# yqtianust/FeatureNet

Hardware: AMD Instinct MI355X
Metric: samples/sec (64^3 voxel, 24-class) train (higher is better)
Workload: dtype bf16; 1 GPU; model=FeatureNet-3D, global_batch=128, per_gpu_batch=128, input=64^3x1 voxels, classes=24, parallelism=dp1, impl=native, optimizer=adam, graph=True

## Files before the change

featurenet_amd/csrc/kernels/bind.cpp:

```cpp
#include <hip/hip_runtime.h>
#include <pybind11/pybind11.h>
#include <pybind11/stl.h>

#include <stdexcept>
#include <string>
#include <vector>

namespace py = pybind11;

extern "C" {
int fn_igemm_fwd(const void*, const void*, const float*, void*, float*, const int*, const int*, long long, int, int,
                 int, int, int, hipStream_t, float*, int);
int fn_igemm_fwd_splits(long long, int, int);
int fn_igemm_fwd_mblocks(long long);
int fn_conv_halo(const void*, const void*, const float*, void*, float*, const int*, const int*, int, int, int*,
                 hipStream_t);
long long fn_conv_halo_lds(const int*, int);
int fn_conv_halo_workers(const int*, int);
int fn_pw_fwd(const void*, const void*, const float*, void*, long long, int, int, int, hipStream_t, const float*,
              const float*, int, const void*, const float*, const float*, float*, int);
int fn_seghead_part_len();
int fn_part_reduce(const float*, float*, long long, int, int, hipStream_t);
int fn_seghead_blocks(long long);
int fn_seghead_loss(const void*, const float*, const float*, const void*, const float*, const void*, void*, float*,
// ... 66 lines not shown
int fn_dense_wgrad_slices(int, int, int);
int fn_s2d_weight_map(const float*, float*, const int*, int, hipStream_t);
int fn_subpixel_wmap(const float*, float*, int, int, int, hipStream_t);
int fn_halo_pack_w(const float*, void*, int, int, int, int, int, int, int, hipStream_t);
int fn_igemm_pack_w(const float*, void*, int, int, int, int, int, int, int, int, int, hipStream_t);
int fn_pack_w_multi(const long long*, int, hipStream_t);
int fn_igemm_wgrad(const void*, const void*, float*, const int*, const int*, long long, int, int, int, int,
                   hipStream_t, int, int, const void*, int, float*, int, float*);
long long fn_igemm_wgrad_part(int, int, int, int, int, int, int);
int fn_colstats(const void*, const void*, const float*, const float*, const float*, const float*, float*, long long,
                int, int, int, int, hipStream_t);
int fn_bn_finalize(const float*, int, int, double, const float*, const float*, float*, float*, float, float, float*,
                   float*, float*, float*, int, hipStream_t);
int fn_bn_apply(const void*, const float*, const float*, void*, long long, int, int, hipStream_t, void*);
int fn_bn_wdot(const float*, const float*, float*, int, int, int, hipStream_t);
int fn_bn_bwd_prep(const float*, int, const float*, int, int, double, const float*, const float*, const float*,
                   const float*, const float*, const float*, float*, float*, const void*, const void*, long long,
                   hipStream_t);
int fn_bn_bwd_apply_k_blocks(long long, int);
int fn_bn_bwd_apply_k(const void*, const void*, const float*, const float*, const float*, const float*, void*,
                      long long, int, float*, int, hipStream_t);
int fn_bn_bwd_apply(const void*, const void*, const float*, const float*, const float*, const float*, const float*,
                    const float*, void*, long long, int, float, int, hipStream_t);
int fn_bn_bwd_apply_s2d(const void*, const void*, const float*, const float*, const float*, const float*,
                        const float*, const float*, void*, int, int, int, int, int, float, int, hipStream_t);
int fn_pool_fwd(const void*, void*, const float*, const float*, const int*, int, int, int, hipStream_t);
int fn_pool_bwd(const void*, const void*, void*, const float*, const float*, const int*, int, int, int, hipStream_t);
int fn_pool_bwd_stats_blocks(const int*);
int fn_colstats_blocks(long long, int, int, int);
int fn_pool_bn_bwd_apply(const void*, const void*, const float*, const float*, const float*, const float*,
                         const float*, const float*, void*, const int*, int, float, hipStream_t);
int fn_pool_bwd_stats(const void*, const void*, void*, const float*, const float*, const int*, int, float*,
                      hipStream_t);
int fn_softmax_xent_blocks(long long, int);
int fn_upsample2x(const void*, void*, int, int, int, int, int, int, hipStream_t);
int fn_softmax_xent_rows(const void*, int, const long long*, float*, void*, int*, long long, int, float, float,
                         hipStream_t);
int fn_adam_flat_dev(float*, const float*, float*, float*, void*, long long, const float*, int*, int, hipStream_t);
int fn_adam_flat(float*, const float*, float*, float*, void*, long long, float, float, float, float, float, float,
                 float, float, int, hipStream_t);
int fn_sgd_flat(float*, const float*, float*, void*, long long, float, float, float, int, float, hipStream_t);
int fn_bias_act(const void*, const float*, void*, long long, int, int, hipStream_t);
int fn_act_bwd(const void*, const void*, void*, long long, int, hipStream_t);
int fn_dropout(const void*, void*, long long, float, unsigned, unsigned, hipStream_t);
int fn_cast_f32_bf16(const float*, void*, long long, hipStream_t);
int fn_scale_unless_one(void*, int, const float*, long long, hipStream_t);
int fn_copy2(void*, const void*, long long, void*, const void*, long long, hipStream_t);
int fn_cu_occupy(int, int, int, void*, hipStream_t);
int fn_softmax_rows(const float*, float*, long long, int, int, const float*, hipStream_t);
int fn_unpack_bits(const void*, void*, long long, hipStream_t);
int fn_conv_tile(const void*, const void*, const void*, const void*, const void*, const float*, void*, float*,
                 const int*, int, int, int, int, int*, hipStream_t, const void*, const float*, float, void*);
int fn_conv_tile_workers(const int*, int, int);
int fn_conv_tile_slab_rows(const int*, int, int);
void fn_conv_tile_grid_cap(int);
void fn_conv_tile_set_schedule(int);
int fn_conv_tile_schedule();
int fn_conv_tile_f8(const void*, const void*, const void*, const void*, const void*, const float*, const float*, void*,
                    float, const int*, int, int, int, int, int*, hipStream_t, const void*, void*);
int fn_conv_tile_f8_supported(int, int, int);
int fn_conv_wtile(const void*, const void*, float*, float*, const void*, const void*, const void*, const int*, int, int,
                  int*, hipStream_t, const float*, float*, const float*, int);
int fn_conv_wtile_supported(int, int);
int fn_conv_wtile_prologue_built();
int fn_tile_pack_w(const float*, void*, int, int, int, int, int, int, int, int, int, hipStream_t);
int fn_tile_pack_w2(const float*, void*, void*, int, int, int, const int*, const int*, hipStream_t);
// ... 832 lines not shown
  m.def("pool_fwd", [check_pool](uintptr_t x, uintptr_t out, uintptr_t scale, uintptr_t shift, std::vector<int> geom,
                       int is_max, int count_pad, int act, uintptr_t st, std::vector<long long> ext) {
    need(geom, 17, "pool_fwd");
    check_pool(geom, ext, "pool_fwd");
    chk(fn_pool_fwd(P<const void*>(x), P<void*>(out), P<const float*>(scale), P<const float*>(shift), geom.data(),
                    is_max, count_pad, act, S(st)),
        "pool_fwd");
  }, py::arg("x"), py::arg("out"), py::arg("scale"), py::arg("shift"), py::arg("geom"), py::arg("is_max"),
     py::arg("count_pad"), py::arg("act"), py::arg("st"), py::arg("ext") = std::vector<long long>());
  m.def("pool_bwd", [check_pool](uintptr_t dout, uintptr_t x, uintptr_t dx, uintptr_t scale, uintptr_t shift,
                       std::vector<int> geom, int is_max, int count_pad, int act, uintptr_t st,
                       std::vector<long long> ext) {
    need(geom, 17, "pool_bwd");
    check_pool(geom, ext, "pool_bwd");
    chk(fn_pool_bwd(P<const void*>(dout), P<const void*>(x), P<void*>(dx), P<const float*>(scale),
                    P<const float*>(shift), geom.data(), is_max, count_pad, act, S(st)),
        "pool_bwd");
  }, py::arg("dout"), py::arg("x"), py::arg("dx"), py::arg("scale"), py::arg("shift"), py::arg("geom"),
     py::arg("is_max"), py::arg("count_pad"), py::arg("act"), py::arg("st"), py::arg("ext") = std::vector<long long>());
  m.def("pool_bwd_stats_blocks", [](std::vector<int> geom) {
    need(geom, 17, "pool_bwd_stats_blocks");
    return fn_pool_bwd_stats_blocks(geom.data());
  });
  m.def("pool_bwd_stats", [check_pool](uintptr_t dout, uintptr_t x, uintptr_t dx, uintptr_t scale, uintptr_t shift,
                             std::vector<int> geom, int act, uintptr_t part, uintptr_t st, std::vector<long long> ext) {
    need(geom, 17, "pool_bwd_stats");
    check_pool(geom, ext, "pool_bwd_stats");
    fits(ext, 2, 2LL * fn_pool_bwd_stats_blocks(geom.data()) * geom[4], "pool_bwd_stats", "part");
    chk(fn_pool_bwd_stats(P<const void*>(dout), P<const void*>(x), P<void*>(dx), P<const float*>(scale),
                          P<const float*>(shift), geom.data(), act, P<float*>(part), S(st)),
        "pool_bwd_stats");
  }, py::arg("dout"), py::arg("x"), py::arg("dx"), py::arg("scale"), py::arg("shift"), py::arg("geom"),
     py::arg("act"), py::arg("part"), py::arg("st"), py::arg("ext") = std::vector<long long>());
  m.def("pool_bn_bwd_apply", [check_pool](uintptr_t dout, uintptr_t y, uintptr_t scale, uintptr_t shift,
                                uintptr_t mean, uintptr_t invstd, uintptr_t dbeta, uintptr_t dgamma, uintptr_t dy,
                                std::vector<int> geom, int act, float inv_count, uintptr_t st,
                                std::vector<long long> ext) {
    need(geom, 17, "pool_bn_bwd_apply");
    check_pool(geom, ext, "pool_bn_bwd_apply");
    chk(fn_pool_bn_bwd_apply(P<const void*>(dout), P<const void*>(y), P<const float*>(scale), P<const float*>(shift),
                             P<const float*>(mean), P<const float*>(invstd), P<const float*>(dbeta),
                             P<const float*>(dgamma), P<void*>(dy), geom.data(), act, inv_count, S(st)),
        "pool_bn_bwd_apply");
  }, py::arg("dout"), py::arg("y"), py::arg("scale"), py::arg("shift"), py::arg("mean"), py::arg("invstd"),
     py::arg("dbeta"), py::arg("dgamma"), py::arg("dy"), py::arg("geom"), py::arg("act"), py::arg("inv_count"),
     py::arg("st"), py::arg("ext") = std::vector<long long>());
  m.def("upsample2x", [](uintptr_t x, uintptr_t y, int N, int D, int H, int W, int C, int backward, uintptr_t st) {
    chk(fn_upsample2x(P<const void*>(x), P<void*>(y), N, D, H, W, C, backward, S(st)), "upsample2x");
  });
  m.def("softmax_xent_blocks", [](long long B, int NC) { return fn_softmax_xent_blocks(B, NC); });
  m.def("softmax_xent_rows", [](uintptr_t logits, int in_bf16, uintptr_t labels, uintptr_t block_loss,
                                uintptr_t dlogits, uintptr_t correct, long long B, int NC, float gscale,
                                float smoothing, uintptr_t st) {
    chk(fn_softmax_xent_rows(P<const void*>(logits), in_bf16, P<const long long*>(labels), P<float*>(block_loss),
                             P<void*>(dlogits), P<int*>(correct), B, NC, gscale, smoothing, S(st)),
        "softmax_xent_rows");
  });
  m.def("softmax_rows", [](uintptr_t x, uintptr_t y, long long M, int N, int backward, uintptr_t g, uintptr_t st,
                           std::vector<long long> ext) {
    fits(ext, 0, M * N, "softmax_rows", "x");
    fits(ext, 1, M * N, "softmax_rows", "y");
    if (backward) fits(ext, 2, M * N, "softmax_rows", "g");
    chk(fn_softmax_rows(P<const float*>(x), P<float*>(y), M, N, backward, P<const float*>(g), S(st)), "softmax_rows");
  });
  m.def("cu_occupy", [](int nwg, int usec, int lds, uintptr_t sink, uintptr_t st) {
    chk(fn_cu_occupy(nwg, usec, lds, P<void*>(sink), S(st)), "cu_occupy");
// ... 44 lines not shown
```

featurenet_amd/csrc/kernels/bn_pool.hip:

```cpp
#include "common.h"

#include <algorithm>
#include <type_traits>

template <int VW>
__device__ __forceinline__ void block_moments_to_part(const float (&s0)[VW], const float (&s1)[VW], bool active, int C,
                                                      float* __restrict__ part) {
  __shared__ float red[256][2 * VW + 1];
  const int tid = threadIdx.x;
  const int cpr = C / VW, rpp = 256 / cpr;
#pragma unroll
  for (int j = 0; j < VW; ++j) { red[tid][j] = active ? s0[j] : 0.f; red[tid][VW + j] = active ? s1[j] : 0.f; }
  __syncthreads();
  for (int c = tid; c < C; c += 256) {
    const int chk = c / VW, j = c % VW;
    float a = 0.f, b = 0.f;
    for (int i = 0; i < rpp; ++i) { a += red[i * cpr + chk][j]; b += red[i * cpr + chk][VW + j]; }
    part[(long long)blockIdx.x * 2 * C + c] = a;
    part[(long long)blockIdx.x * 2 * C + C + c] = b;
  }
}

template <int VW>
__device__ __forceinline__ void bn_bwd_consts(int c0, const float* __restrict__ scale, const float* __restrict__ shift,
// ... 509 lines not shown
          const int iw = ow * g.sw - g.pw + kw;
          if ((unsigned)iw >= (unsigned)g.W) continue;
          ++cnt;
          const long long base = (((n * g.D + id) * g.H + ih) * (long long)g.W + iw) * g.C + ch * VW;
          if constexpr (VW == 8) {
            Pack8 p;
            p.u = *(const uint4*)(x + base);
#pragma unroll
            for (int j = 0; j < 8; ++j) {
              float v = bf2f(p.e[j]);
              if (scale) v = act_fwd(v * scale[ch * 8 + j] + shift[ch * 8 + j], act);
              accv[j] = is_max ? fmaxf(accv[j], v) : accv[j] + v;
            }
          } else {
            const float v = load_pre(x, base, ch, scale, shift, act);
            accv[0] = is_max ? fmaxf(accv[0], v) : accv[0] + v;
          }
        }
      }
    }
    const float div = count_pad ? (float)(g.KD * g.KH * g.KW) : (float)(cnt > 0 ? cnt : 1);
    const long long ob = i * VW;
    if constexpr (VW == 8) {
      Pack8 p;
#pragma unroll
      for (int j = 0; j < 8; ++j) p.e[j] = f2bf(is_max ? accv[j] : accv[j] / div);
      *(uint4*)(out + ob) = p.u;
    } else {
      out[ob] = f2bf(is_max ? accv[0] : accv[0] / div);
    }
  }
}

template <int KD, int ACT = -1>
__global__ __launch_bounds__(256) void pool2_fwd_kernel(const bf16* __restrict__ x, bf16* __restrict__ out,
                                                        const float* __restrict__ scale, const float* __restrict__ shift,
                                                        PoolGeom g, int is_max, int act, int total) {
  const int actc = ACT >= 0 ? ACT : act;
  const int cpr = g.C >> 3;
  const int ch = threadIdx.x % cpr;
  float sc[8], sh[8];
#pragma unroll
  for (int j = 0; j < 8; ++j) {
    sc[j] = scale ? scale[ch * 8 + j] : 1.f;
    sh[j] = scale ? shift[ch * 8 + j] : 0.f;
  }
  const long long rowW = (long long)g.W * g.C, plane = (long long)g.H * rowW;
  auto origin = [&](int ii) -> long long {
    int t = ii / cpr;
    const int ow = t % g.OW; t /= g.OW;
    const int oh = t % g.OH; t /= g.OH;
    const int od = t % g.OD;
    const int n = t / g.OD;
    return ((long long)(n * g.D + od * KD) * g.H + oh * 2) * rowW + (long long)ow * 2 * g.C + ch * 8;
  };
  auto fetch = [&](long long b0, Pack8* p) {
#pragma unroll
    for (int kd = 0; kd < KD; ++kd)
#pragma unroll
      for (int kh = 0; kh < 2; ++kh)
#pragma unroll
        for (int kw = 0; kw < 2; ++kw) p[(kd * 2 + kh) * 2 + kw].u = *(const uint4*)(x + b0 + kd * plane + kh * rowW + kw * g.C);
  };
  const int stride = gridDim.x * 256;
  int i = blockIdx.x * 256 + threadIdx.x;
  Pack8 p[KD * 4];
  if (i < total) fetch(origin(i), p);
  while (i < total) {
    const int inx = i + stride;
    Pack8 p2[KD * 4];
    fetch(origin(inx < total ? inx : i), p2);
    Pack8 o;
#pragma unroll
    for (int j = 0; j < 8; ++j) {
      float acc = is_max ? -INFINITY : 0.f;
#pragma unroll
      for (int w = 0; w < KD * 4; ++w) {
        float v = bf2f(p[w].e[j]);
        if (scale) v = act_fwd(v * sc[j] + sh[j], actc);
        acc = is_max ? fmaxf(acc, v) : acc + v;
      }
      o.e[j] = f2bf(is_max ? acc : acc * (1.f / (KD * 4)));
    }
    *(uint4*)(out + (long long)i * 8) = o.u;
#pragma unroll
    for (int w = 0; w < KD * 4; ++w) p[w] = p2[w];
    i = inx;
  }
}

template <int VW>
__global__ __launch_bounds__(256) void pool_bwd_kernel(const bf16* __restrict__ dout, const bf16* __restrict__ x,
                                                       bf16* __restrict__ dx, const float* __restrict__ scale,
                                                       const float* __restrict__ shift, PoolGeom g, int is_max,
                                                       int count_pad, int act) {
  const int cpr = g.C / VW;
  const long long total = (long long)g.N * g.D * g.H * g.W * cpr;
  for (long long i = blockIdx.x * 256LL + threadIdx.x; i < total; i += (long long)gridDim.x * 256) {
    const int ch = (int)(i % cpr);
    long long t = i / cpr;
    const int iw = (int)(t % g.W); t /= g.W;
    const int ih = (int)(t % g.H); t /= g.H;
    const int id = (int)(t % g.D);
    const long long n = t / g.D;
    float gacc[VW];
    float self[VW];
#pragma unroll
    for (int j = 0; j < VW; ++j) {
      gacc[j] = 0.f;
      const int c = ch * VW + j;
      self[j] = is_max ? load_pre(x, i * VW + j, c, scale, shift, act) : 0.f;
    }
    const int od0 = max(0, (id + g.pd - g.KD + g.sd) / g.sd), od1 = min(g.OD - 1, (id + g.pd) / g.sd);
    const int oh0 = max(0, (ih + g.ph - g.KH + g.sh) / g.sh), oh1 = min(g.OH - 1, (ih + g.ph) / g.sh);
    const int ow0 = max(0, (iw + g.pw - g.KW + g.sw) / g.sw), ow1 = min(g.OW - 1, (iw + g.pw) / g.sw);
    for (int od = od0; od <= od1; ++od)
      for (int oh = oh0; oh <= oh1; ++oh)
// ... 183 lines not shown
      if (w < win) qy[w].u = *(const uint4*)(y + b0 + wofs[w]);
  };
  const I stride = (I)gridDim.x * 256;
  I i = (I)blockIdx.x * 256 + threadIdx.x;
  Pack8 pg, py[8];
  if (i < total) fetch(i, pg, py);
  while (i < total) {
    const I inx = i + stride;
    Pack8 pg2, py2[8];
    fetch(inx < total ? inx : i, pg2, py2);
#pragma unroll
    for (int j = 0; j < 8; ++j) {
      float best = -INFINITY, yarg = 0.f;
#pragma unroll
      for (int w = 0; w < 8; ++w) {
        if (w < win) {
          const float yv = bf2f(py[w].e[j]);
          const float v = act_fwd(yv * sc[j] + sh[j], actc);
          if (v > best) { best = v; yarg = yv; }
        }
      }
      const float gv = bf2f(pg.e[j]) * act_bwd_from_out(best, actc);
      s0[j] += gv;
      s1[j] += gv * yarg;
    }
    pg = pg2;
#pragma unroll
    for (int w = 0; w < 8; ++w) py[w] = py2[w];
    i = inx;
  }
  block_moments_to_part<8>(s0, s1, true, g.C, part);
}

template <typename I, int ACT = -1>
__global__ __launch_bounds__(256) void pool_bn_bwd_apply_kernel(
    const bf16* __restrict__ dout, const bf16* __restrict__ y, const float* __restrict__ scale,
    const float* __restrict__ shift, const float* __restrict__ mean, const float* __restrict__ invstd,
    const float* __restrict__ dbeta, const float* __restrict__ dgamma, bf16* __restrict__ dy, PoolGeom g, int act,
    float inv_count) {
  const int actc = ACT >= 0 ? ACT : act;
  const int cpr = g.C / 8;
  const I total = (I)g.N * g.OD * g.OH * g.OW * cpr;
  const int win = g.KD * g.KH * g.KW;
  const int ch = (int)(threadIdx.x % cpr);
  float sc[8], sh[8], k2[8], k3[8];
  bn_bwd_consts<8>(ch * 8, scale, shift, mean, invstd, dbeta, dgamma, inv_count, sc, sh, k2, k3);
  I wofs[8];
  pool_win_offsets<I>(g, win, wofs);
  auto origin = [&](I ii) -> I { return pool_win_origin<I>(g, ii, cpr, ch); };
  auto fetch = [&](I ii, I b0, Pack8& q, Pack8* qy) {
    q.u = *(const uint4*)(dout + ii * 8);
#pragma unroll
    for (int w = 0; w < 8; ++w)
      if (w < win) qy[w].u = *(const uint4*)(y + b0 + wofs[w]);
  };
  const I stride = (I)gridDim.x * 256;
  I i = (I)blockIdx.x * 256 + threadIdx.x;
  Pack8 pg, py[8];
  I b0 = 0;
  if (i < total) {
    b0 = origin(i);
    fetch(i, b0, pg, py);
  }
  while (i < total) {
    const I inx = i + stride;
    const I in2 = inx < total ? inx : i;
// ... 186 lines not shown
    const int u = rowlen > 4 * 256 && rowlen <= 5 * 256 ? 5 : (rowlen > 5 * 256 && rowlen <= 8 * 256 ? 8 : 4);
    bool launched = false;
    with_int_of<ACT_RELU, ACT_NONE>(act, [&](auto A) {
      with_int_of<0, 1, 2, 3, 4, 5>(lc, [&](auto L) {
        launched = with_int_of<4, 5, 8>(u, [&](auto U) {
          hipLaunchKernelGGL((bn_bwd_apply_s2d_rows_kernel<A(), L(), U()>), dim3(grid), dim3(256), 0, st,
                             (const bf16*)dz, (const bf16*)y, scale, shift, mean, invstd, dbeta, dgamma, (bf16*)dsh, N,
                             FD, FH, FW, C, inv_count);
        });
      });
    });
    if (!launched) return -2;
    FN_CHECK_LAUNCH();
    return 0;
  }
  with_act(act, [&](auto A) {
    hipLaunchKernelGGL((bn_bwd_apply_s2d_kernel<A()>), dim3(ew_blocks(nvec)), dim3(256), 0, st, (const bf16*)dz,
                       (const bf16*)y, scale, shift, mean, invstd, dbeta, dgamma, (bf16*)dsh, N, FD, FH, FW, C, inv_count);
  });
  FN_CHECK_LAUNCH();
  return 0;
}

static PoolGeom pool_geom(const int* g) {
  PoolGeom p;
  p.N = g[0]; p.D = g[1]; p.H = g[2]; p.W = g[3]; p.C = g[4];
  p.OD = g[5]; p.OH = g[6]; p.OW = g[7];
  p.KD = g[8]; p.KH = g[9]; p.KW = g[10];
  p.sd = g[11]; p.sh = g[12]; p.sw = g[13];
  p.pd = g[14]; p.ph = g[15]; p.pw = g[16];
  return p;
}

extern "C" int fn_pool_fwd(const void* x, void* out, const float* scale, const float* shift, const int* geom17,
                           int is_max, int count_pad, int act, hipStream_t st) {
  PoolGeom g = pool_geom(geom17);
  const long long outs = (long long)g.N * g.OD * g.OH * g.OW;
  const bool win2 = g.KH == 2 && g.KW == 2 && (g.KD == 2 || g.KD == 1) && g.sd == g.KD && g.sh == 2 && g.sw == 2 &&
                    g.pd == 0 && g.ph == 0 && g.pw == 0 && g.D >= g.OD * g.KD && g.H >= g.OH * 2 &&
                    g.W >= g.OW * 2 && chunk_fixed(g.C) && outs * (g.C / 8) + 256LL * 8192 < (1LL << 31);
  if (win2) {
    const int total = (int)(outs * (g.C / 8));
    with_int_of<2, 1>(g.KD, [&](auto K) {
      with_act_rn(scale ? act : ACT_NONE, [&](auto A) {
        static const int res = bn_resident_blocks((const void*)pool2_fwd_kernel<K(), A()>);
        hipLaunchKernelGGL((pool2_fwd_kernel<K(), A()>), dim3(resident_grid((total + 255) / 256, res)), dim3(256), 0,
                           st, (const bf16*)x, (bf16*)out, scale, shift, g, is_max, act, total);
      });
    });
  } else
    with_vw(g.C % 8 == 0, [&](auto VW) {
      hipLaunchKernelGGL(pool_fwd_kernel<VW()>, dim3(ew_blocks(outs * (g.C / VW()))), dim3(256), 0, st, (const bf16*)x,
                         (bf16*)out, scale, shift, g, is_max, count_pad, act);
    });
  FN_CHECK_LAUNCH();
  return 0;
}

static bool pool_i32(const PoolGeom& g) {
  const long long ins = (long long)g.N * g.D * g.H * g.W * g.C;
  const long long outs = (long long)g.N * g.OD * g.OH * g.OW * g.C;
  return ins + 256LL * 8192 * 8 < (1LL << 31) && outs + 256LL * 8192 * 8 < (1LL << 31);
}

static bool pool_tiled(const PoolGeom& g) {
  return g.sd == g.KD && g.sh == g.KH && g.sw == g.KW && g.pd == 0 && g.ph == 0 && g.pw == 0 &&
         g.D == g.OD * g.KD && g.H == g.OH * g.KH && g.W == g.OW * g.KW;
}

static bool pool_bwd_stats_ok(const PoolGeom& g) { return pool_tiled(g) && chunk_fixed(g.C); }

extern "C" int fn_pool_bwd_stats_blocks(const int* geom17) {
  const PoolGeom g = pool_geom(geom17);
  if (!pool_bwd_stats_ok(g)) return 0;
  int res = 0;
  if (g.KD * g.KH * g.KW <= 8) {
    static const int r = bn_resident_blocks((const void*)pool_bn_moments8_kernel<int>);
    res = r;
  }
  return resident_rows(((long long)g.N * g.OD * g.OH * g.OW * (g.C / 8) + 255) / 256, res);
}

extern "C" int fn_pool_bwd_stats(const void* dout, const void* x, void* dx, const float* scale, const float* shift,
                                 const int* geom17, int act, float* part, hipStream_t st) {
  const PoolGeom g = pool_geom(geom17);
  const int nb = fn_pool_bwd_stats_blocks(geom17);
  if (nb <= 0 || !scale || !shift || !part) return -2;
  if (!dx && g.KD * g.KH * g.KW <= 8) {
    with_index(pool_i32(g), [&](auto I) {
      with_act_rn(act, [&](auto A) {
        hipLaunchKernelGGL((pool_bn_moments8_kernel<decltype(I), A()>), dim3(nb), dim3(256), 0, st, (const bf16*)dout,
                           (const bf16*)x, scale, shift, g, act, part);
      });
    });
  } else
    hipLaunchKernelGGL((pool_bwd_tiled_kernel<8, true>), dim3(nb), dim3(256), 0, st, (const bf16*)dout, (const bf16*)x,
                       (bf16*)dx, scale, shift, g, 1, act, part);
  FN_CHECK_LAUNCH();
  return 0;
}

extern "C" int fn_pool_bn_bwd_apply(const void* dout, const void* y, const float* scale, const float* shift,
                                    const float* mean, const float* invstd, const float* dbeta, const float* dgamma,
                                    void* dy, const int* geom17, int act, float inv_count, hipStream_t st) {
  const PoolGeom g = pool_geom(geom17);
  if (!pool_tiled(g) || !chunk_fixed(g.C) || g.KD * g.KH * g.KW > 8) return -2;
  const long long outs = (long long)g.N * g.OD * g.OH * g.OW;
  static const int res = bn_resident_blocks((const void*)pool_bn_bwd_apply_kernel<int>);
  const unsigned nb = resident_grid((outs * (g.C / 8) + 255) / 256, res);
  with_index(pool_i32(g), [&](auto I) {
    with_act_rn(act, [&](auto A) {
      hipLaunchKernelGGL((pool_bn_bwd_apply_kernel<decltype(I), A()>), dim3(nb), dim3(256), 0, st, (const bf16*)dout,
                         (const bf16*)y, scale, shift, mean, invstd, dbeta, dgamma, (bf16*)dy, g, act, inv_count);
    });
  });
  FN_CHECK_LAUNCH();
  return 0;
}

extern "C" int fn_pool_bwd(const void* dout, const void* x, void* dx, const float* scale, const float* shift,
                           const int* geom17, int is_max, int count_pad, int act, hipStream_t st) {
  PoolGeom g = pool_geom(geom17);
  if (pool_tiled(g)) {
    const long long outs = (long long)g.N * g.OD * g.OH * g.OW;
    with_vw(g.C % 8 == 0, [&](auto VW) {
      hipLaunchKernelGGL(pool_bwd_tiled_kernel<VW()>, dim3(ew_blocks(outs * (g.C / VW()))), dim3(256), 0, st,
                         (const bf16*)dout, (const bf16*)x, (bf16*)dx, scale, shift, g, is_max, act);
    });
    FN_CHECK_LAUNCH();
    return 0;
  }
  const long long ins = (long long)g.N * g.D * g.H * g.W;
  with_int_of<8, 2, 1>(g.C % 8 == 0 ? 8 : (g.C % 2 == 0 ? 2 : 1), [&](auto VW) {
    hipLaunchKernelGGL(pool_bwd_kernel<VW()>, dim3(ew_blocks(ins * (g.C / VW()))), dim3(256), 0, st, (const bf16*)dout,
// ... 39 lines not shown
```

featurenet_amd/models/layers.py:

```python
from __future__ import annotations

import math

import torch
from torch import nn

from .. import ops
from ..ops.spec import ConvSpec, PoolSpec, _triple, to5d_shape


def glorot_uniform_(w: torch.Tensor, fan_in: int, fan_out: int, gen: torch.Generator | None = None) -> torch.Tensor:
    lim = math.sqrt(6.0 / (fan_in + fan_out))
    with torch.no_grad():
        return w.uniform_(-lim, lim, generator=gen)


def he_normal_(w: torch.Tensor, fan_in: int, gen: torch.Generator | None = None) -> torch.Tensor:
    with torch.no_grad():
        return w.normal_(0.0, math.sqrt(2.0 / fan_in), generator=gen)


class Conv(nn.Module):

    def __init__(self, cin: int, cout: int, kernel, stride=1, padding="valid", dilation=1, bn: bool = False,
# ... 22 lines not shown
            self.register_buffer("running_mean", torch.zeros(cout))
            self.register_buffer("running_var", torch.ones(cout))
            self.bn_momentum, self.bn_eps = bn_momentum, bn_eps
        self._spec_cache: dict = {}

    def specs(self, shape5):
        s = self._spec_cache.get(shape5)
        if s is None:
            cs = ConvSpec.make(shape5, self.cout, self.kernel, self.stride, self.padding, self.dilation,
                               extra=getattr(self, "extra_pad", (0, 0, 0)))
            ps = None
            if self.pool is not None:
                ps = PoolSpec.make(cs.out_shape5, self.pool, self.pool_stride, self.pool_padding)
            s = (cs, ps)
            self._spec_cache[shape5] = s
        return s

    def forward(self, x: torch.Tensor) -> torch.Tensor:
        in_shape = x.shape
        x5 = x.reshape(to5d_shape(in_shape))
        cs, ps = self.specs(tuple(x5.shape))
        if self.bn and not self.training:
            scale = self.gamma * torch.rsqrt(self.running_var + self.bn_eps)
            w = self.weight * scale.view(-1, 1, 1, 1, 1)
            b = self.beta - self.running_mean * scale
            out = ops.conv(x5, w, b, cs, self.act)
            if ps is not None:
                out = ops.pool(out, ps, self.pool_kind)
        elif self.bn:
            y, slab = ops.conv(x5, self.weight, None, cs, None, want_stats=True)
            if ps is not None:
                out = ops.batchnorm_act_pool(y, self.gamma, self.beta, self.running_mean, self.running_var,
                                             self.training, ps, self.pool_kind, self.bn_momentum, self.bn_eps,
                                             self.act, stats_slab=slab)
            else:
                out = ops.batchnorm_act(y, self.gamma, self.beta, self.running_mean, self.running_var,
                                        self.training, self.bn_momentum, self.bn_eps, self.act, stats_slab=slab)
        else:
            out = ops.conv(x5, self.weight, self.bias, cs, self.act)
            if ps is not None:
                out = ops.pool(out, ps, self.pool_kind)
        n, d, h, w, c = out.shape
        if len(in_shape) == 4:
            return out.reshape(n, h, w, c)
        if len(in_shape) == 3:
            return out.reshape(n, w, c)
        return out

    def flops(self, shape5) -> int:
        cs, _ = self.specs(tuple(shape5))
        return cs.flops()


class Dense(nn.Module):

    def __init__(self, fin: int, fout: int, act=None, bias: bool = True, init: str = "glorot"):
        super().__init__()
        self.fin, self.fout, self.act = fin, fout, act
        self.weight = nn.Parameter(torch.empty(fout, fin))
        if init == "he":
            he_normal_(self.weight, fin)
        else:
            glorot_uniform_(self.weight, fin, fout)
        self.bias = nn.Parameter(torch.zeros(fout)) if bias else None

    def forward(self, x: torch.Tensor, out_fp32: bool = False) -> torch.Tensor:
        return ops.linear(x, self.weight, self.bias, self.act, out_fp32=out_fp32)
# ... 89 lines not shown
```

featurenet_amd/ops/bn.py:

```python
from __future__ import annotations

import torch

from .. import _native
from ..training.flat import grad_target
from . import bnfuse
from . import reference as ref
from .spec import PoolSpec, act_code


def _stats_slab(y2: torch.Tensor) -> torch.Tensor:
    M, C = y2.shape
    nb = _native.kernels().colstats_blocks(M, C, 0, 0)
    part = torch.empty(nb, 2, C, dtype=torch.float32, device=y2.device)
    _native.kernels().colstats(y2.data_ptr(), 0, 0, 0, 0, 0, part.data_ptr(), M, C, 0, 0, nb, _native.stream(y2))
    return part


def _finalize_fwd(slab, count, gamma, beta, rmean, rvar, momentum, eps, update_running=True):
    C = slab.shape[-1]
    out = torch.empty(4, C, dtype=torch.float32, device=slab.device)
    _native.kernels().bn_finalize(
        slab.data_ptr(), slab.shape[0], C, float(count), _native.ptr(gamma), _native.ptr(beta),
        _native.ptr(rmean) if update_running else 0, _native.ptr(rvar) if update_running else 0,
# ... 90 lines not shown
                                   C, act, _native.stream(y), _native.ptr(mask), 0 if mask is None else mask.numel())
        if tag and act in (0, 1):
            bnfuse.tag_output(z, y, prm, act, mask)
        ctx.mask = mask
        ctx.save_for_backward(y, prm)
        ctx.act, ctx.training = act, training
        ctx.has_gamma, ctx.has_beta = gamma is not None, beta is not None
        ctx.params = (beta, gamma)
        return z

    @staticmethod
    def backward(ctx, dz):
        y, prm = ctx.saved_tensors
        C = y.shape[-1]
        y2 = y.reshape(-1, C)
        dz2 = dz.contiguous().to(torch.bfloat16).reshape(-1, C)
        part = bnfuse.take(dz2, y) if ctx.training else None
        ctx.mask = None
        if isinstance(part, tuple) and ctx.needs_input_grad[0]:
            dy, dbeta, dgamma = _bwd_identity(dz2, y2, prm, *ctx.params, gslab=part[1], wpart=part[2])
            return (dy.reshape(y.shape), dgamma if ctx.has_gamma else None, dbeta if ctx.has_beta else None,
                    None, None, None, None, None, None, None, None)
        dbeta = dgamma = None
        if ctx.training or ctx.needs_input_grad[1] or ctx.needs_input_grad[2]:
            dbeta, dgamma = _bwd_param_grads(dz2, y2, prm, ctx.act, *ctx.params)
        dy = _bwd_input(dz2, y2, prm, dbeta, dgamma, ctx.act, ctx.training) if ctx.needs_input_grad[0] else None
        return (None if dy is None else dy.reshape(y.shape), dgamma if ctx.has_gamma else None,
                dbeta if ctx.has_beta else None, None, None, None, None, None, None, None, None)


class BatchNormActPoolFn(torch.autograd.Function):

    @staticmethod
    def forward(ctx, y, gamma, beta, slab, rmean, rvar, training, momentum, eps, act, pspec, is_max, count_pad):
        C = y.shape[-1]
        y2 = y.reshape(-1, C)
        if training:
            if slab is None:
                slab = _stats_slab(y2)
            prm = _finalize_fwd(slab, y2.shape[0], gamma, beta, rmean, rvar, momentum, eps)
        else:
            prm = _eval_params(gamma, beta, rmean, rvar, eps, C, y.device)
        p = torch.empty(pspec.out_shape5, dtype=torch.bfloat16, device=y.device)
        _native.kernels().pool_fwd(y.data_ptr(), p.data_ptr(), prm[2].data_ptr(), prm[3].data_ptr(), pspec.geom17(),
                                   int(is_max), int(count_pad), act, _native.stream(y), [y.numel(), p.numel()])
        ctx.save_for_backward(y, prm)
        ctx.act, ctx.training, ctx.pspec, ctx.is_max, ctx.count_pad = act, training, pspec, is_max, count_pad
        ctx.has_gamma, ctx.has_beta = gamma is not None, beta is not None
        ctx.params = (beta, gamma)
        return p

    @staticmethod
    def backward(ctx, dp):
        y, prm = ctx.saved_tensors
        C = y.shape[-1]
        dp = dp.contiguous().to(torch.bfloat16)
        K = _native.kernels()
        geom = ctx.pspec.geom17()
        nb = K.pool_bwd_stats_blocks(geom) if (ctx.is_max and ctx.training and bnfuse.pool_stats_enabled()) else 0
        part = None
        ps = ctx.pspec
        if nb > 0 and bnfuse.pool_apply_enabled() and ps.KD * ps.KH * ps.KW <= 8 and C % 8 == 0:
            part = torch.empty(nb, 2, C, dtype=torch.float32, device=y.device)
            K.pool_bwd_stats(dp.data_ptr(), y.data_ptr(), 0, prm[2].data_ptr(), prm[3].data_ptr(), geom, ctx.act,
                             part.data_ptr(), _native.stream(y), [y.numel(), dp.numel(), part.numel()])
            y2 = y.reshape(-1, C)
            dbeta, dgamma = _bwd_param_grads(None, y2, prm, ctx.act, *ctx.params, part=part)
            dy = None
            if ctx.needs_input_grad[0]:
                dy = torch.empty_like(y)
                K.pool_bn_bwd_apply(dp.data_ptr(), y.data_ptr(), prm[2].data_ptr(), prm[3].data_ptr(),
                                    prm[0].data_ptr(), prm[1].data_ptr(), dbeta.data_ptr(), dgamma.data_ptr(),
                                    dy.data_ptr(), geom, ctx.act, 1.0 / y2.shape[0], _native.stream(y),
                                    [y.numel(), dp.numel()])
            return (dy, dgamma if ctx.has_gamma else None, dbeta if ctx.has_beta else None) + (None,) * 10
        dz = torch.empty_like(y)
        if nb > 0:
            part = torch.empty(nb, 2, C, dtype=torch.float32, device=y.device)
            K.pool_bwd_stats(dp.data_ptr(), y.data_ptr(), dz.data_ptr(), prm[2].data_ptr(), prm[3].data_ptr(), geom,
                             ctx.act, part.data_ptr(), _native.stream(y), [y.numel(), dp.numel(), part.numel()])
        else:
            K.pool_bwd(dp.data_ptr(), y.data_ptr(), dz.data_ptr(), prm[2].data_ptr(), prm[3].data_ptr(), geom,
                       int(ctx.is_max), int(ctx.count_pad), ctx.act, _native.stream(y), [y.numel(), dp.numel()])
        y2, dz2 = y.reshape(-1, C), dz.reshape(-1, C)
        dbeta = dgamma = None
        if ctx.training or ctx.needs_input_grad[1] or ctx.needs_input_grad[2]:
            dbeta, dgamma = _bwd_param_grads(dz2, y2, prm, ctx.act, *ctx.params, part=part)
        dy = _bwd_input(dz2, y2, prm, dbeta, dgamma, ctx.act, ctx.training) if ctx.needs_input_grad[0] else None
        return (None if dy is None else dy.reshape(y.shape), dgamma if ctx.has_gamma else None,
                dbeta if ctx.has_beta else None) + (None,) * 10


def batchnorm_act(y5, gamma, beta, running_mean, running_var, training: bool, momentum: float = 0.1,
                  eps: float = 1e-5, act=None, stats_slab=None):
    if _native.use_native(y5):
        tag = training and torch.is_grad_enabled() and (y5.requires_grad or any(
            p is not None and p.requires_grad for p in (gamma, beta)))
        return BatchNormActFn.apply(y5.to(torch.bfloat16).contiguous(), gamma, beta, stats_slab, running_mean,
                                    running_var, training, momentum, eps, act_code(act), tag)
    return ref.batchnorm_act(y5, gamma, beta, running_mean, running_var, training, momentum, eps, act)


def batchnorm_act_pool(y5, gamma, beta, running_mean, running_var, training: bool, pspec: PoolSpec,
                       kind: str = "max", momentum: float = 0.1, eps: float = 1e-5, act=None, stats_slab=None,
                       count_pad: bool = False):
    if _native.use_native(y5):
        return BatchNormActPoolFn.apply(y5.to(torch.bfloat16).contiguous(), gamma, beta, stats_slab, running_mean,
                                        running_var, training, momentum, eps, act_code(act), pspec, kind == "max",
                                        count_pad)
    z = ref.batchnorm_act(y5, gamma, beta, running_mean, running_var, training, momentum, eps, act)
    return ref.pool(z, pspec, kind, count_pad)


class BatchNormActPointwiseFn(torch.autograd.Function):

    @staticmethod
    def forward(ctx, y, gamma, beta, slab, rmean, rvar, momentum, eps, act, w, b):
        from .conv import pw_fwd

        C = y.shape[-1]
        y2 = y.reshape(-1, C)
        if slab is None:
            slab = _stats_slab(y2)
        prm = _finalize_fwd(slab, y2.shape[0], gamma, beta, rmean, rvar, momentum, eps)
        N = w.shape[0]
        w2 = w.detach().reshape(N, C)
        bias = b.detach().float().contiguous() if b is not None else None
        out = pw_fwd(y2, w2, bias, 0, pro=(prm[2], prm[3], act))
        ctx.save_for_backward(y, prm, w)
        ctx.act, ctx.has_b, ctx.bparam = act, b is not None, b
        ctx.params = (beta, gamma)
        return out.reshape(*y.shape[:-1], N)

    @staticmethod
    def backward(ctx, dout):
        from .conv import native_colsum, pw_fwd, pw_wgrad

        y, prm, w = ctx.saved_tensors
        C = y.shape[-1]
        N = w.shape[0]
        y2 = y.reshape(-1, C)
        d2 = dout.contiguous().to(torch.bfloat16).reshape(-1, N)
# ... 36 lines not shown
```

featurenet_amd/ops/bnfuse.py:

```python
from __future__ import annotations

import os
import threading
import weakref

import torch

_LOCK = threading.Lock()
_FWD: dict = {}
_BWD: dict = {}


def identity_enabled() -> bool:
    return os.environ.get("FN_BN_IDENTITY", "1") != "0"


def identity_ok(C: int, act: int) -> bool:
    return identity_enabled() and act == 1 and C in (32, 64)


def pool_stats_enabled() -> bool:
    return os.environ.get("FN_POOL_BN_STATS", "1") != "0"


def pool_apply_enabled() -> bool:
    return os.environ.get("FN_POOL_BN_APPLY", "1") != "0"


def _purge(d: dict, limit: int = 256) -> None:
    if len(d) > limit:
        for k in [k for k, v in d.items() if v[0]() is None]:
            d.pop(k, None)


def tag_output(z: torch.Tensor, y: torch.Tensor, prm: torch.Tensor, act: int, mask=None) -> None:
    if mask is None:
        return
    with _LOCK:
        _purge(_FWD)
        _FWD[z.data_ptr()] = (weakref.ref(z), weakref.ref(y), weakref.ref(prm), act,
                              weakref.ref(mask) if mask is not None else None)


def source_of(x: torch.Tensor):
    e = _FWD.get(x.data_ptr())
    if e is None:
        return None
    z, y, prm = e[0](), e[1](), e[2]()
    if z is None or y is None or prm is None or z.numel() != x.numel() or not x.is_contiguous():
        return None
    mask = e[4]() if e[4] is not None else None
    return y, prm, e[3], mask


def offer(dz: torch.Tensor, slab, y: torch.Tensor) -> None:
    with _LOCK:
        _purge(_BWD)
        _BWD[dz.data_ptr()] = (weakref.ref(dz), slab, weakref.ref(y), dz._version)

# ... 13 lines not shown
```

Measured before the change: 28480 samples/s.

## Save argmax pre-BN values in pooled forward to compute backward BN moments cheaply

The fused BN+act+maxpool forward now also writes, for each pooled output, the pre-normalization value that won the max (an optional index buffer is supported but not used). In backward, the BN gradient moments are computed from the pooled gradient and this saved tensor, avoiding a re-read of the full-resolution input and re-evaluation of pooling windows. This costs one extra pooled-sized bf16 write in forward plus extra live memory, and the tie-breaking may differ from the existing recompute path.

```diff
diff --git a/featurenet_amd/csrc/kernels/bind.cpp b/featurenet_amd/csrc/kernels/bind.cpp
--- a/featurenet_amd/csrc/kernels/bind.cpp
+++ b/featurenet_amd/csrc/kernels/bind.cpp
@@ -122,6 +122,9 @@
                          const float*, const float*, void*, const int*, int, float, hipStream_t);
 int fn_pool_bwd_stats(const void*, const void*, void*, const float*, const float*, const int*, int, float*,
                       hipStream_t);
+int fn_pool_fwd_save_ok(const int*, int);
+int fn_pool_fwd_save(const void*, void*, void*, void*, const float*, const float*, const int*, int, hipStream_t);
+int fn_pool_moments_saved(const void*, const void*, const float*, const float*, const int*, int, float*, hipStream_t);
 int fn_softmax_xent_blocks(long long, int);
 int fn_upsample2x(const void*, void*, int, int, int, int, int, int, hipStream_t);
 int fn_softmax_xent_rows(const void*, int, const long long*, float*, void*, int*, long long, int, float, float,
@@ -1020,6 +1023,34 @@
         "pool_bwd_stats");
   }, py::arg("dout"), py::arg("x"), py::arg("dx"), py::arg("scale"), py::arg("shift"), py::arg("geom"),
      py::arg("act"), py::arg("part"), py::arg("st"), py::arg("ext") = std::vector<long long>());
+  m.def("pool_fwd_save_ok", [](std::vector<int> geom, int act) {
+    need(geom, 17, "pool_fwd_save_ok");
+    return fn_pool_fwd_save_ok(geom.data(), act);
+  });
+  m.def("pool_fwd_save", [check_pool](uintptr_t x, uintptr_t out, uintptr_t ymax, uintptr_t idx, uintptr_t scale,
+                            uintptr_t shift, std::vector<int> geom, int act, uintptr_t st,
+                            std::vector<long long> ext) {
+    need(geom, 17, "pool_fwd_save");
+    check_pool(geom, ext, "pool_fwd_save");
+    const long long outs = prod({geom[0], geom[5], geom[6], geom[7], geom[4]});
+    fits(ext, 2, outs, "pool_fwd_save", "ymax");
+    if (idx) fits(ext, 3, outs, "pool_fwd_save", "idx");
+    chk(fn_pool_fwd_save(P<const void*>(x), P<void*>(out), P<void*>(ymax), P<void*>(idx), P<const float*>(scale),
+                         P<const float*>(shift), geom.data(), act, S(st)),
+        "pool_fwd_save");
+  });
+  m.def("pool_moments_saved", [](uintptr_t dout, uintptr_t ymax, uintptr_t scale, uintptr_t shift,
+                                 std::vector<int> geom, int act, uintptr_t part, uintptr_t st,
+                                 std::vector<long long> ext) {
+    need(geom, 17, "pool_moments_saved");
+    const long long outs = prod({geom[0], geom[5], geom[6], geom[7], geom[4]});
+    fits(ext, 0, outs, "pool_moments_saved", "dout");
+    fits(ext, 1, outs, "pool_moments_saved", "ymax");
+    fits(ext, 2, 2LL * fn_pool_bwd_stats_blocks(geom.data()) * geom[4], "pool_moments_saved", "part");
+    chk(fn_pool_moments_saved(P<const void*>(dout), P<const void*>(ymax), P<const float*>(scale),
+                              P<const float*>(shift), geom.data(), act, P<float*>(part), S(st)),
+        "pool_moments_saved");
+  });
   m.def("pool_bn_bwd_apply", [check_pool](uintptr_t dout, uintptr_t y, uintptr_t scale, uintptr_t shift,
                                 uintptr_t mean, uintptr_t invstd, uintptr_t dbeta, uintptr_t dgamma, uintptr_t dy,
                                 std::vector<int> geom, int act, float inv_count, uintptr_t st,
diff --git a/featurenet_amd/csrc/kernels/bn_pool.hip b/featurenet_amd/csrc/kernels/bn_pool.hip
--- a/featurenet_amd/csrc/kernels/bn_pool.hip
+++ b/featurenet_amd/csrc/kernels/bn_pool.hip
@@ -565,10 +565,12 @@
   }
 }
 
-template <int KD, int ACT = -1>
+template <int KD, int ACT = -1, bool SAVE = false>
 __global__ __launch_bounds__(256) void pool2_fwd_kernel(const bf16* __restrict__ x, bf16* __restrict__ out,
                                                         const float* __restrict__ scale, const float* __restrict__ shift,
-                                                        PoolGeom g, int is_max, int act, int total) {
+                                                        PoolGeom g, int is_max, int act, int total,
+                                                        bf16* __restrict__ ymax = nullptr,
+                                                        unsigned char* __restrict__ idx = nullptr) {
   const int actc = ACT >= 0 ? ACT : act;
   const int cpr = g.C >> 3;
   const int ch = threadIdx.x % cpr;
@@ -604,18 +606,34 @@
     Pack8 p2[KD * 4];
     fetch(origin(inx < total ? inx : i), p2);
     Pack8 o;
+    [[maybe_unused]] Pack8 oy;
+    [[maybe_unused]] unsigned long long oi = 0ull;
 #pragma unroll
     for (int j = 0; j < 8; ++j) {
       float acc = is_max ? -INFINITY : 0.f;
+      [[maybe_unused]] float best = -INFINITY;
+      [[maybe_unused]] bf16 yb = f2bf(0.f);
+      [[maybe_unused]] int ab = 0;
 #pragma unroll
       for (int w = 0; w < KD * 4; ++w) {
         float v = bf2f(p[w].e[j]);
         if (scale) v = act_fwd(v * sc[j] + sh[j], actc);
         acc = is_max ? fmaxf(acc, v) : acc + v;
+        if constexpr (SAVE) {
+          if (v > best) { best = v; yb = p[w].e[j]; ab = w; }
+        }
       }
       o.e[j] = f2bf(is_max ? acc : acc * (1.f / (KD * 4)));
+      if constexpr (SAVE) {
+        oy.e[j] = yb;
+        oi |= (unsigned long long)ab << (8 * j);
+      }
     }
     *(uint4*)(out + (long long)i * 8) = o.u;
+    if constexpr (SAVE) {
+      *(uint4*)(ymax + (long long)i * 8) = oy.u;
+      if (idx) *(unsigned long long*)(idx + (long long)i * 8) = oi;
+    }
 #pragma unroll
     for (int w = 0; w < KD * 4; ++w) p[w] = p2[w];
     i = inx;
@@ -865,6 +883,48 @@
   block_moments_to_part<8>(s0, s1, true, g.C, part);
 }
 
+template <int ACT = -1>
+__global__ __launch_bounds__(256) void pool_moments_saved_kernel(const bf16* __restrict__ dout,
+                                                                 const bf16* __restrict__ ymax,
+                                                                 const float* __restrict__ scale,
+                                                                 const float* __restrict__ shift, long long total,
+                                                                 int C, int act, float* __restrict__ part) {
+  const int actc = ACT >= 0 ? ACT : act;
+  const int cpr = C / 8;
+  const int ch = (int)(threadIdx.x % cpr);
+  float sc[8], sh[8], s0[8], s1[8];
+#pragma unroll
+  for (int j = 0; j < 8; ++j) {
+    sc[j] = scale[ch * 8 + j];
+    sh[j] = shift[ch * 8 + j];
+    s0[j] = s1[j] = 0.f;
+  }
+  const long long stride = (long long)gridDim.x * 256;
+  for (long long i = (long long)blockIdx.x * 256 + threadIdx.x; i < total; i += 4 * stride) {
+    Pack8 pg[4], py[4];
+#pragma unroll
+    for (int u = 0; u < 4; ++u) {
+      const long long iu = i + u * stride < total ? i + u * stride : i;
+      pg[u].u = *(const uint4*)(dout + iu * 8);
+      py[u].u = *(const uint4*)(ymax + iu * 8);
+    }
+#pragma unroll
+    for (int u = 0; u < 4; ++u) {
+      if (i + u * stride < total) {
+#pragma unroll
+        for (int j = 0; j < 8; ++j) {
+          const float yarg = bf2f(py[u].e[j]);
+          const float best = act_fwd(yarg * sc[j] + sh[j], actc);
+          const float gv = bf2f(pg[u].e[j]) * act_bwd_from_out(best, actc);
+          s0[j] += gv;
+          s1[j] += gv * yarg;
+        }
+      }
+    }
+  }
+  block_moments_to_part<8>(s0, s1, true, C, part);
+}
+
 template <typename I, int ACT = -1>
 __global__ __launch_bounds__(256) void pool_bn_bwd_apply_kernel(
     const bf16* __restrict__ dout, const bf16* __restrict__ y, const float* __restrict__ scale,
@@ -1117,14 +1177,18 @@
   return p;
 }
 
+static bool pool_win2(const PoolGeom& g) {
+  const long long outs = (long long)g.N * g.OD * g.OH * g.OW;
+  return g.KH == 2 && g.KW == 2 && (g.KD == 2 || g.KD == 1) && g.sd == g.KD && g.sh == 2 && g.sw == 2 && g.pd == 0 &&
+         g.ph == 0 && g.pw == 0 && g.D >= g.OD * g.KD && g.H >= g.OH * 2 && g.W >= g.OW * 2 && chunk_fixed(g.C) &&
+         outs * (g.C / 8) + 256LL * 8192 < (1LL << 31);
+}
+
 extern "C" int fn_pool_fwd(const void* x, void* out, const float* scale, const float* shift, const int* geom17,
                            int is_max, int count_pad, int act, hipStream_t st) {
   PoolGeom g = pool_geom(geom17);
   const long long outs = (long long)g.N * g.OD * g.OH * g.OW;
-  const bool win2 = g.KH == 2 && g.KW == 2 && (g.KD == 2 || g.KD == 1) && g.sd == g.KD && g.sh == 2 && g.sw == 2 &&
-                    g.pd == 0 && g.ph == 0 && g.pw == 0 && g.D >= g.OD * g.KD && g.H >= g.OH * 2 &&
-                    g.W >= g.OW * 2 && chunk_fixed(g.C) && outs * (g.C / 8) + 256LL * 8192 < (1LL << 31);
-  if (win2) {
+  if (pool_win2(g)) {
     const int total = (int)(outs * (g.C / 8));
     with_int_of<2, 1>(g.KD, [&](auto K) {
       with_act_rn(scale ? act : ACT_NONE, [&](auto A) {
@@ -1138,6 +1202,30 @@
       hipLaunchKernelGGL(pool_fwd_kernel<VW()>, dim3(ew_blocks(outs * (g.C / VW()))), dim3(256), 0, st, (const bf16*)x,
                          (bf16*)out, scale, shift, g, is_max, count_pad, act);
     });
+  FN_CHECK_LAUNCH();
+  return 0;
+}
+
+static bool pool_tiled(const PoolGeom& g);
+
+extern "C" int fn_pool_fwd_save_ok(const int* geom17, int act) {
+  const PoolGeom g = pool_geom(geom17);
+  return pool_win2(g) && pool_tiled(g) && (act == ACT_RELU || act == ACT_NONE);
+}
+
+extern "C" int fn_pool_fwd_save(const void* x, void* out, void* ymax, void* idx, const float* scale,
+                                const float* shift, const int* geom17, int act, hipStream_t st) {
+  const PoolGeom g = pool_geom(geom17);
+  if (!fn_pool_fwd_save_ok(geom17, act) || !scale || !shift || !ymax) return -2;
+  const int total = (int)((long long)g.N * g.OD * g.OH * g.OW * (g.C / 8));
+  with_int_of<2, 1>(g.KD, [&](auto K) {
+    with_int_of<ACT_RELU, ACT_NONE>(act, [&](auto A) {
+      static const int res = bn_resident_blocks((const void*)pool2_fwd_kernel<K(), A(), true>);
+      hipLaunchKernelGGL((pool2_fwd_kernel<K(), A(), true>), dim3(resident_grid((total + 255) / 256, res)), dim3(256),
+                         0, st, (const bf16*)x, (bf16*)out, scale, shift, g, 1, act, total, (bf16*)ymax,
+                         (unsigned char*)idx);
+    });
+  });
   FN_CHECK_LAUNCH();
   return 0;
 }
@@ -1185,6 +1273,20 @@
   return 0;
 }
 
+extern "C" int fn_pool_moments_saved(const void* dout, const void* ymax, const float* scale, const float* shift,
+                                     const int* geom17, int act, float* part, hipStream_t st) {
+  const PoolGeom g = pool_geom(geom17);
+  const int nb = fn_pool_bwd_stats_blocks(geom17);
+  if (nb <= 0 || !fn_pool_fwd_save_ok(geom17, act) || !scale || !shift || !part || !ymax) return -2;
+  const long long total = (long long)g.N * g.OD * g.OH * g.OW * (g.C / 8);
+  with_int_of<ACT_RELU, ACT_NONE>(act, [&](auto A) {
+    hipLaunchKernelGGL((pool_moments_saved_kernel<A()>), dim3(nb), dim3(256), 0, st, (const bf16*)dout,
+                       (const bf16*)ymax, scale, shift, total, g.C, act, part);
+  });
+  FN_CHECK_LAUNCH();
+  return 0;
+}
+
 extern "C" int fn_pool_bn_bwd_apply(const void* dout, const void* y, const float* scale, const float* shift,
                                     const float* mean, const float* invstd, const float* dbeta, const float* dgamma,
                                     void* dy, const int* geom17, int act, float inv_count, hipStream_t st) {
diff --git a/featurenet_amd/models/layers.py b/featurenet_amd/models/layers.py
--- a/featurenet_amd/models/layers.py
+++ b/featurenet_amd/models/layers.py
@@ -78,7 +78,7 @@
             if ps is not None:
                 out = ops.batchnorm_act_pool(y, self.gamma, self.beta, self.running_mean, self.running_var,
                                              self.training, ps, self.pool_kind, self.bn_momentum, self.bn_eps,
-                                             self.act, stats_slab=slab)
+                                             self.act, stats_slab=slab, save_argmax=True)
             else:
                 out = ops.batchnorm_act(y, self.gamma, self.beta, self.running_mean, self.running_var,
                                         self.training, self.bn_momentum, self.bn_eps, self.act, stats_slab=slab)
diff --git a/featurenet_amd/ops/bn.py b/featurenet_amd/ops/bn.py
--- a/featurenet_amd/ops/bn.py
+++ b/featurenet_amd/ops/bn.py
@@ -146,7 +146,8 @@
 class BatchNormActPoolFn(torch.autograd.Function):
 
     @staticmethod
-    def forward(ctx, y, gamma, beta, slab, rmean, rvar, training, momentum, eps, act, pspec, is_max, count_pad):
+    def forward(ctx, y, gamma, beta, slab, rmean, rvar, training, momentum, eps, act, pspec, is_max, count_pad,
+                save_argmax=False):
         C = y.shape[-1]
         y2 = y.reshape(-1, C)
         if training:
@@ -156,8 +157,17 @@
         else:
             prm = _eval_params(gamma, beta, rmean, rvar, eps, C, y.device)
         p = torch.empty(pspec.out_shape5, dtype=torch.bfloat16, device=y.device)
-        _native.kernels().pool_fwd(y.data_ptr(), p.data_ptr(), prm[2].data_ptr(), prm[3].data_ptr(), pspec.geom17(),
-                                   int(is_max), int(count_pad), act, _native.stream(y), [y.numel(), p.numel()])
+        K = _native.kernels()
+        ymax = None
+        if save_argmax and bnfuse.pool_stats_enabled() and bnfuse.pool_apply_enabled() \
+                and K.pool_fwd_save_ok(pspec.geom17(), act):
+            ymax = torch.empty_like(p)
+            K.pool_fwd_save(y.data_ptr(), p.data_ptr(), ymax.data_ptr(), 0, prm[2].data_ptr(), prm[3].data_ptr(),
+                            pspec.geom17(), act, _native.stream(y), [y.numel(), p.numel(), ymax.numel(), 0])
+        else:
+            K.pool_fwd(y.data_ptr(), p.data_ptr(), prm[2].data_ptr(), prm[3].data_ptr(), pspec.geom17(),
+                       int(is_max), int(count_pad), act, _native.stream(y), [y.numel(), p.numel()])
+        ctx.ymax = ymax
         ctx.save_for_backward(y, prm)
         ctx.act, ctx.training, ctx.pspec, ctx.is_max, ctx.count_pad = act, training, pspec, is_max, count_pad
         ctx.has_gamma, ctx.has_beta = gamma is not None, beta is not None
@@ -176,8 +186,13 @@
         ps = ctx.pspec
         if nb > 0 and bnfuse.pool_apply_enabled() and ps.KD * ps.KH * ps.KW <= 8 and C % 8 == 0:
             part = torch.empty(nb, 2, C, dtype=torch.float32, device=y.device)
-            K.pool_bwd_stats(dp.data_ptr(), y.data_ptr(), 0, prm[2].data_ptr(), prm[3].data_ptr(), geom, ctx.act,
-                             part.data_ptr(), _native.stream(y), [y.numel(), dp.numel(), part.numel()])
+            if ctx.ymax is not None:
+                K.pool_moments_saved(dp.data_ptr(), ctx.ymax.data_ptr(), prm[2].data_ptr(), prm[3].data_ptr(), geom,
+                                     ctx.act, part.data_ptr(), _native.stream(y),
+                                     [dp.numel(), ctx.ymax.numel(), part.numel()])
+            else:
+                K.pool_bwd_stats(dp.data_ptr(), y.data_ptr(), 0, prm[2].data_ptr(), prm[3].data_ptr(), geom, ctx.act,
+                                 part.data_ptr(), _native.stream(y), [y.numel(), dp.numel(), part.numel()])
             y2 = y.reshape(-1, C)
             dbeta, dgamma = _bwd_param_grads(None, y2, prm, ctx.act, *ctx.params, part=part)
             dy = None
@@ -187,7 +202,7 @@
                                     prm[0].data_ptr(), prm[1].data_ptr(), dbeta.data_ptr(), dgamma.data_ptr(),
                                     dy.data_ptr(), geom, ctx.act, 1.0 / y2.shape[0], _native.stream(y),
                                     [y.numel(), dp.numel()])
-            return (dy, dgamma if ctx.has_gamma else None, dbeta if ctx.has_beta else None) + (None,) * 10
+            return (dy, dgamma if ctx.has_gamma else None, dbeta if ctx.has_beta else None) + (None,) * 11
         dz = torch.empty_like(y)
         if nb > 0:
             part = torch.empty(nb, 2, C, dtype=torch.float32, device=y.device)
@@ -202,7 +217,7 @@
             dbeta, dgamma = _bwd_param_grads(dz2, y2, prm, ctx.act, *ctx.params, part=part)
         dy = _bwd_input(dz2, y2, prm, dbeta, dgamma, ctx.act, ctx.training) if ctx.needs_input_grad[0] else None
         return (None if dy is None else dy.reshape(y.shape), dgamma if ctx.has_gamma else None,
-                dbeta if ctx.has_beta else None) + (None,) * 10
+                dbeta if ctx.has_beta else None) + (None,) * 11
 
 
 def batchnorm_act(y5, gamma, beta, running_mean, running_var, training: bool, momentum: float = 0.1,
@@ -217,11 +232,13 @@
 
 def batchnorm_act_pool(y5, gamma, beta, running_mean, running_var, training: bool, pspec: PoolSpec,
                        kind: str = "max", momentum: float = 0.1, eps: float = 1e-5, act=None, stats_slab=None,
-                       count_pad: bool = False):
+                       count_pad: bool = False, save_argmax: bool = False):
     if _native.use_native(y5):
+        save = bool(save_argmax and training and kind == "max" and torch.is_grad_enabled()
+                    and bnfuse.pool_save_enabled())
         return BatchNormActPoolFn.apply(y5.to(torch.bfloat16).contiguous(), gamma, beta, stats_slab, running_mean,
                                         running_var, training, momentum, eps, act_code(act), pspec, kind == "max",
-                                        count_pad)
+                                        count_pad, save)
     z = ref.batchnorm_act(y5, gamma, beta, running_mean, running_var, training, momentum, eps, act)
     return ref.pool(z, pspec, kind, count_pad)
 
diff --git a/featurenet_amd/ops/bnfuse.py b/featurenet_amd/ops/bnfuse.py
--- a/featurenet_amd/ops/bnfuse.py
+++ b/featurenet_amd/ops/bnfuse.py
@@ -25,6 +25,10 @@
 
 def pool_apply_enabled() -> bool:
     return os.environ.get("FN_POOL_BN_APPLY", "1") != "0"
+
+
+def pool_save_enabled() -> bool:
+    return os.environ.get("FN_POOL_SAVE", "1") != "0"
 
 
 def _purge(d: dict, limit: int = 256) -> None:
```

Measured after the change: 28590 samples/s (median of 6 runs). Within noise of the previous version (+0.4%).
